# ZechengLi19/CIM

Hardware: AMD Instinct MI355X
Metric: images/sec training step (ResNet-50 VOC, ~1k proposals/img) at 1/2/4/8 GPU (higher is better)
Workload: dtype fp32

## Files before the change

cim_amd/_lib.py:

```python
import ctypes
import os

from ctypes import c_float, c_int, c_longlong, c_void_p

HERE = os.path.dirname(os.path.abspath(__file__))
LIB_PATH = os.environ.get("CIM_HIP_LIB") or os.path.join(HERE, "libcim_hip.so")

_P = c_void_p
SIGNATURES = {
    "cim_roi_align_fwd": [_P, _P, _P] + [c_int] * 6 + [c_float, c_int, c_int, _P],
    "cim_roi_align_fwd_ws": [_P, _P, _P] + [c_int] * 6 + [c_float, c_int, c_int, _P, _P],
    "cim_roi_align_maskcat_fwd_ws": [_P, _P, _P, _P] + [c_int] * 6 + [c_float, c_int, c_int, _P, _P],
    "cim_roi_align_wino7_pair_fwd": [_P, _P, _P, _P, _P] + [c_int] * 7 + [c_float, c_int, c_int, _P, _P],
    "cim_roi_align_bwd_ws": [_P, _P, _P] + [c_int] * 6 + [c_float, c_int, c_int, _P, c_int, _P, _P],
    "cim_roi_align_maskcat_bwd_ws": [_P, _P, _P, _P] + [c_int] * 6 + [c_float, c_int, c_int, _P, c_int, _P, _P],
    "cim_roi_align_bwd_workspace": [c_int, c_int, c_int, c_int],
    "cim_roi_align_bwd_scratch": [c_int, c_int, c_int, c_int, c_int],
    "cim_roi_align_bwd": [_P, _P, _P] + [c_int] * 6 + [c_float, c_int, c_int, _P, _P],
    "cim_roi_align_maskcat_fwd": [_P, _P, _P, _P] + [c_int] * 6 + [c_float, c_int, c_int, _P],
    "cim_roi_align_maskcat_bwd": [_P, _P, _P, _P] + [c_int] * 6 + [c_float, c_int, c_int, _P, _P],
    "cim_roi_align_forms": [c_int] * 9 + [_P] * 3,
    "cim_maxpool2d_out_size": [c_int, c_int, c_int, c_int],
    "cim_maxpool2d_fwd": [_P, _P, _P, c_int, c_int, c_int, c_int, c_int, c_int, _P],
    "cim_maxpool2d_bwd": [_P, _P, _P, c_int, c_int, c_int, c_int, c_int, c_int, _P],
    "cim_upsample_nearest_fwd": [_P, _P, c_int, c_int, c_int, c_int, c_int, _P],
    "cim_upsample_nearest_bwd": [_P, _P, c_int, c_int, c_int, c_int, _P],
    "cim_image_prep": [_P, c_int, c_int, _P, c_int, c_int, c_longlong, c_int, ctypes.c_double, c_int, _P, _P],
    "cim_mask_pack": [_P, _P, c_int, c_int, _P],
    "cim_mask_iou_pair": [_P, c_int, c_int, _P, _P, _P, _P],
    "cim_asy_flag": [_P, c_int, c_float, _P, _P],
    "cim_asy_prep": [_P, c_int, _P, c_int, _P, _P, _P],
    "cim_mining_step": [_P, _P, _P],
    "cim_mining_lds_bytes": [c_int, c_int],
    "cim_mining_sync_bytes": [],
    "cim_gemm_small_splits": [c_int, c_int, c_int],
    "cim_gemm_small_f32": [_P, _P, _P] + [c_int] * 8 + [_P, _P, _P, _P, _P, c_float, _P, c_int, c_int, _P, _P],
    "cim_conv1x1_bwd_workspace": [c_int, c_int, c_int, c_int],
    "cim_conv1x1_bn_act_bwd": [_P] * 8 + [c_float, c_int] + [_P] * 5 + [c_int] * 4 + [_P, _P, _P, _P, _P, c_int] + [c_int, _P, _P, c_float] + [_P] * 4 + [c_int],
    "cim_bn_part_finish": [_P, c_int, _P],
    "cim_conv3x3_nchw_splits": [c_int] * 5,
    "cim_conv3x3_nchw_f32": [_P, _P, _P] + [c_int] * 6 + [_P, _P, _P, _P, _P, c_float, _P, c_int, c_int, _P, _P],
    "cim_conv7x7_nchw_f32": [_P, _P, _P] + [c_int] * 5 + [_P, _P, _P, _P, c_float, c_int, _P],
    "cim_conv3x3_nchw_bwd_workspace": [c_int] * 6,
    "cim_conv3x3_dx_parts": [c_int] * 3,
    "cim_conv3x3_nchw_bn_act_bwd": [_P] * 8 + [c_float, c_int] + [_P] * 5 + [c_int] * 7 + [_P, _P, _P, _P, _P, c_int] + [c_int, _P, _P, c_float] + [_P] * 4,
    "cim_conv3x3_wt_multi": [_P, c_int, _P],
    "cim_bn_act_fwd": [_P, _P, _P, _P, _P, _P, c_float, _P, c_int, c_int, c_int, c_int, _P],
    "cim_bn_act_bwd_chunks": [c_int, c_int, c_int],
    "cim_bn_act_bwd": [_P, _P, _P, _P, _P, _P, c_float, _P, _P, _P, _P, c_int, c_int, c_int, c_int, _P],
    "cim_sgd_multi": [_P, _P, c_int, c_float, c_int, _P],
    "cim_adam_multi": [_P, _P, c_int, ctypes.c_double, ctypes.c_double, ctypes.c_double, c_int, _P],
    "cim_gemm_pair_splits": [c_int, c_int, c_int],
    "cim_gemm_pair": [_P, _P, _P, _P] + [c_int] * 6 + [c_int, c_int, c_int, c_int, _P, _P, _P, _P, c_int, c_int, c_int, _P],
    "cim_gemm_pair_batched": [_P, _P, _P] + [c_int] * 6 + [c_int, c_int, c_int, c_longlong, c_longlong, c_longlong,
                              _P, _P, c_int, c_int, c_int, _P],
    "cim_pair_scales": [_P, c_int, _P, _P, c_int, c_int, _P],
    "cim_pair_split": [_P, _P, c_int, c_int, c_int, c_int, c_int, c_int, c_longlong, c_longlong, _P, _P, _P],
    "cim_pair_amax": [_P, c_longlong, _P, _P],
    "cim_pair_masked_stats": [_P, _P, c_int, c_int, _P, _P, _P],
    "cim_wino7_flatten_bwd_dy_pair": [_P, _P, _P, _P, _P, _P, _P, c_int, c_int, c_int, _P],
    "cim_wino7_pair_scales": [_P, c_int, _P, c_int, _P, _P],
    "cim_wino7_input_pair": [_P, _P, _P, c_int, c_int, c_int, _P],
    "cim_wino7_filter_pair": [_P, _P, _P, c_int, c_int, _P],
    "cim_wino7_dy_pair": [_P, _P, _P, c_int, c_int, c_int, c_int, _P],
    "cim_wino7_output_amax": [_P, _P, _P, c_int, c_int, c_int, _P, _P],
    "cim_flatten_chw_pair": [_P, _P, _P, c_int, c_int, c_int, c_int, _P],
    "cim_flatten_chw_bwd_bias": [_P, _P, _P, _P, c_int, c_int, c_int, _P],
    "cim_wino_dx_adjoint_output": [_P, _P, c_int, c_int, c_int, c_int, _P],
    "cim_wino7_dx_maskfold": [_P, _P, _P, c_int, c_int, _P],
    "cim_wino_wgrad_output": [_P, _P, c_int, c_int, c_int, _P],
    "cim_losses_fwd": [_P, _P],
    "cim_linear_bias_f32": [_P, _P, _P, _P, c_int, c_int, c_int, c_int, _P, _P],
    "cim_loss_finish": [_P, c_int, _P, _P],
    "cim_loss_grad_combine": [_P] * 8 + [c_int, c_int, c_int, _P],
    "cim_head_act_fwd": [_P, _P, _P, c_int, c_int, c_int, _P],
    "cim_head_act_bwd": [_P, _P, _P, _P, c_int, c_int, c_int, _P],
    "cim_detect_ws_bytes": [c_int, c_int],
    "cim_detect_nms_limit": [_P, c_int, _P, c_int, c_int, c_float, c_float, c_int, _P, _P, _P, _P, _P],
    "cim_detect_corloc": [_P, c_int, c_int, c_int, _P, _P],
    "cim_segm_words": [c_int, c_int],
    "cim_segm_pack": [_P, _P, c_longlong, c_int, c_int, c_int, _P, _P],
    "cim_segm_area": [_P, c_int, c_int, _P, _P],
    "cim_segm_rle_count": [_P, c_int, c_int, c_int, _P, _P],
    "cim_segm_rle_write": [_P, c_int, c_int, c_int, _P, _P, _P, _P],
    "cim_segm_rle_decode_ws_bytes": [c_longlong],
    "cim_segm_rle_decode": [_P, _P, _P, c_int, c_int, c_int, _P, _P, _P],
    "cim_segm_image_ws_bytes": [c_int, c_int, c_longlong],
    "cim_segm_record_bytes": [c_int, c_int, c_int, c_int],
    "cim_segm_eval_image": [_P, c_int, _P, c_int, c_int, _P, _P, c_int, c_int, c_int, c_longlong, _P, _P, _P, c_int, _P, c_int,
                            _P, _P, _P],
# ... 77 lines not shown
```

cim_amd/csrc/common.h:

```cpp
#pragma once
#include <hip/hip_runtime.h>
#include <hip/hip_fp16.h>
#include <stdint.h>
#include <stdio.h>

namespace cim {

void set_error(const char* fmt, ...);

static inline hipStream_t as_stream(void* s) { return reinterpret_cast<hipStream_t>(s); }

static inline float round_to_f16(float thr) { return (float)(_Float16)thr; }

#define CIM_CHECK_ARG(cond)                                                     \
    do {                                                                        \
        if (!(cond)) {                                                          \
            cim::set_error("%s: bad argument: %s", __func__, #cond);            \
            return -1;                                                          \
        }                                                                       \
    } while (0)

#define CIM_CHECK_LAUNCH()                                                      \
    do {                                                                        \
        hipError_t e_ = hipGetLastError();                                      \
        if (e_ != hipSuccess) {                                                 \
            cim::set_error("%s: %s", __func__, hipGetErrorString(e_));          \
            return (int)e_;                                                     \
        }                                                                       \
    } while (0)

#define CIM_CHECK_HIP(call)                                                     \
    do {                                                                        \
        hipError_t e_ = (call);                                                 \
        if (e_ != hipSuccess) {                                                 \
            cim::set_error("%s: %s", __func__, hipGetErrorString(e_));          \
            return (int)e_;                                                     \
        }                                                                       \
    } while (0)

typedef _Float16 pair_f16x2 __attribute__((ext_vector_type(2)));
typedef float pair_f32x2 __attribute__((ext_vector_type(2)));
__device__ __forceinline__ void pair_split2(float a, float b, unsigned& h, unsigned& l) {
    const pair_f32x2 v = {a, b};
    const pair_f16x2 hv = __builtin_convertvector(v, pair_f16x2);
    const pair_f32x2 r = {a - (float)hv.x, b - (float)hv.y};
    h = __builtin_bit_cast(unsigned, hv);
    l = __builtin_bit_cast(unsigned, __builtin_convertvector(r, pair_f16x2));
}
__device__ __forceinline__ float pair_scale_of(unsigned amax_bits) {
    const int e = (int)((amax_bits >> 23) & 0xffu);
    int b = 268 - e;
    if (b > 253) b = 253;
    if (e == 0 || e == 255) b = 127;
    return __uint_as_float((unsigned)b << 23);
}

__device__ __forceinline__ void amax_publish(unsigned* word, unsigned wave_max) {
    if (wave_max > __hip_atomic_load(word, __ATOMIC_RELAXED, __HIP_MEMORY_SCOPE_AGENT)) atomicMax(word, wave_max);
}

__device__ __forceinline__ float h2f(uint16_t bits) {
    return __half2float(__ushort_as_half(bits));
}

}
```

cim_amd/csrc/gemm_pair.hip:

```cpp
#include "common.h"
#include <type_traits>
#include "../../include/cim_hip.h"

namespace {

using f32x16 = __attribute__((ext_vector_type(16))) float;
using f16x8 = __attribute__((ext_vector_type(8))) _Float16;
typedef short s16x4 __attribute__((__vector_size__(4 * sizeof(short))));
typedef short s16x8 __attribute__((__vector_size__(8 * sizeof(short))));

#ifndef CIM_PAIR_EXP
#define CIM_PAIR_EXP 0
#endif
static_assert(CIM_PAIR_EXP == 0 || (CIM_PAIR_EXP >= 3 && CIM_PAIR_EXP <= 5), "CIM_PAIR_EXP: 0 (product), 3, 4 or 5");
constexpr bool ABL_NO_LOOP_DMA = CIM_PAIR_EXP == 3 || CIM_PAIR_EXP == 5;
constexpr bool ABL_NO_LOOP_READS = CIM_PAIR_EXP == 4 || CIM_PAIR_EXP == 5;

constexpr int BM = 256, BN = 256, BK = 32;
constexpr int NW = 8, NT = 64 * NW;
constexpr int WNC = 4;
constexpr int WM = 128, WN = BN / WNC, MI = 4, NI = WN / 32;
constexpr int IPW = 32 / NW;
constexpr int OPER = 256 * BK * 4;
constexpr int SLAB = 2 * OPER;
// ... 578 lines not shown
using cim::pair_split2;
using cim::pair_scale_of;

__global__ __launch_bounds__(256) void pair_masked_stats_kernel(const float* __restrict__ dy, const float* __restrict__ y, int rows,
                                                                int cols, float* __restrict__ part, unsigned* __restrict__ amax) {
    __shared__ float4 red[16][16];
    const int cx = threadIdx.x & 15, ry = threadIdx.x >> 4;
    const int col = blockIdx.x * 64 + cx * 4, r0 = blockIdx.y * 64;
    float4 s = make_float4(0.f, 0.f, 0.f, 0.f);
    unsigned m = 0;
    if (col < cols) {
#pragma unroll
        for (int i = 0; i < 4; ++i) {
            const int r = r0 + ry * 4 + i;
            if (r < rows) {
                const float4 g = *reinterpret_cast<const float4*>(dy + (size_t)r * cols + col);
                const float4 v = *reinterpret_cast<const float4*>(y + (size_t)r * cols + col);
                const float4 z = make_float4(v.x > 0.f ? g.x : 0.f, v.y > 0.f ? g.y : 0.f, v.z > 0.f ? g.z : 0.f, v.w > 0.f ? g.w : 0.f);
                s.x += z.x; s.y += z.y; s.z += z.z; s.w += z.w;
                m = max(m, abs_bits_max4(z));
            }
        }
    }
    if (part != nullptr) red[ry][cx] = s;
    block_amax_publish(amax, m);
    if (part == nullptr) return;
    if (ry == 0 && col < cols) {
        float4 t = red[0][cx];
#pragma unroll
        for (int k = 1; k < 16; ++k) { const float4 u = red[k][cx]; t.x += u.x; t.y += u.y; t.z += u.z; t.w += u.w; }
        *reinterpret_cast<float4*>(part + (size_t)blockIdx.y * cols + col) = t;
    }
}
__global__ void pair_scales_kernel(const unsigned* __restrict__ amax, int n_amax, const float* __restrict__ factor,
                                   float* __restrict__ scale, int n, int reduce_all) {
    const int i = blockIdx.x * blockDim.x + threadIdx.x;
    unsigned bits = 0;
    if (reduce_all) {
        for (int t = threadIdx.x & 63; t < n_amax; t += 64) bits = max(bits, amax[t] & 0x7fffffffu);
        bits = wave_max_u32(bits);
    }
    if (i >= n) return;
    float a = __uint_as_float(reduce_all ? bits : amax[min(i, n_amax - 1)]);
    if (factor != nullptr) a *= factor[i];
    scale[i] = pair_scale_of(__float_as_uint(a));
}

__global__ __launch_bounds__(256) void pair_split_kernel(const float* __restrict__ X, char* __restrict__ P, int rows,
                                                         int rows_pad, int cols, int ld, int ldp, long long x_bs,
                                                         long long p_bs, const float* __restrict__ scale,
                                                         const float* __restrict__ relu_y) {
    const int chunks = cols >> 3;
    const long long idx = (long long)blockIdx.x * 256 + threadIdx.x;
    if (idx >= (long long)rows_pad * chunks) return;
    const int r = (int)(idx / chunks), c = (int)(idx % chunks);
    const int z = blockIdx.y;
    uint4 h = make_uint4(0, 0, 0, 0), l = make_uint4(0, 0, 0, 0);
    if (r < rows) {
        const float s = scale[z];
        const float* src = X + (size_t)z * x_bs + (size_t)r * ld + c * 8;
        float4 a = *reinterpret_cast<const float4*>(src), b = *reinterpret_cast<const float4*>(src + 4);
        if (relu_y != nullptr) {
            const float* ys = relu_y + (size_t)z * x_bs + (size_t)r * ld + c * 8;
            const float4 ya = *reinterpret_cast<const float4*>(ys), yb = *reinterpret_cast<const float4*>(ys + 4);
            a = make_float4(ya.x > 0.f ? a.x : 0.f, ya.y > 0.f ? a.y : 0.f, ya.z > 0.f ? a.z : 0.f, ya.w > 0.f ? a.w : 0.f);
            b = make_float4(yb.x > 0.f ? b.x : 0.f, yb.y > 0.f ? b.y : 0.f, yb.z > 0.f ? b.z : 0.f, yb.w > 0.f ? b.w : 0.f);
        }
        pair_split2(a.x * s, a.y * s, h.x, l.x);
        pair_split2(a.z * s, a.w * s, h.y, l.y);
        pair_split2(b.x * s, b.y * s, h.z, l.z);
        pair_split2(b.z * s, b.w * s, h.w, l.w);
    }
    char* dst = P + ((size_t)z * p_bs + (size_t)r * ldp + c * 8) * 4;
    *reinterpret_cast<uint4*>(dst) = h;
    *reinterpret_cast<uint4*>(dst + 16) = l;
}

__global__ __launch_bounds__(256) void pair_amax_kernel(const float* __restrict__ X, long long n4, int tail, unsigned* __restrict__ out) {
    unsigned m = 0;
    if (blockIdx.x == 0 && (int)threadIdx.x < tail) m = abs_bits(X[n4 * 4 + threadIdx.x]);
    for (long long i = (long long)blockIdx.x * 256 + threadIdx.x; i < n4; i += (long long)gridDim.x * 256) {
        const uint4 v = *reinterpret_cast<const uint4*>(X + i * 4);
        m = max(m, abs_bits_max4(v));
    }
    block_amax_publish(out, m);
}

template <int AL, int BL, bool RING>
int launch_pair(PairArgs g, int splits, float* workspace, hipStream_t st, int max_workgroups, int products) {
    static_assert(!RING || (AL == L_MC && BL == L_MC), "the ring kernel is the weight gradients' layout only");
    constexpr int TBM = RING ? RBM : BM, LDSB = RING ? RLDS_BYTES : LDS_BYTES, THREADS = RING ? RNT : NT;
    const int tm = (g.M + TBM - 1) / TBM, tn = (g.N + BN - 1) / BN;
    void (*kern)(const PairArgs);
    if constexpr (RING) kern = products == 1 ? gemm_pair_ring_kernel<true> : gemm_pair_ring_kernel<false>;
    else kern = products == 1 ? gemm_pair_kernel<AL, BL, true> : gemm_pair_kernel<AL, BL, false>;
    hipError_t e = hipFuncSetAttribute(reinterpret_cast<const void*>(kern), hipFuncAttributeMaxDynamicSharedMemorySize, LDSB);
    if (e != hipSuccess) return (int)e;
    const int slabs = g.K / BK;
    if (splits < 1) splits = 1;
    if (splits > slabs) splits = slabs;
    g.k_per_split = ((slabs + splits - 1) / splits) * BK;
    splits = (g.K + g.k_per_split - 1) / g.k_per_split;
    float* out = g.C;
    const float* bias = g.bias;
// ... 101 lines not shown
    if (rc) { cim::set_error("cim_gemm_pair: launch setup failed (%d)", rc); return rc; }
    CIM_CHECK_LAUNCH();
    return 0;
}

extern "C" int cim_gemm_pair_batched(const void* A, const void* B, float* C, int M, int N, int K, int lda, int ldb,
                                     int ldc, int a_mcontig, int b_kcontig, int batch, long long a_bs, long long b_bs,
                                     long long c_bs, const float* a_scale, const float* b_scale, int max_workgroups, int products,
                                     int form, void* stream) {
    CIM_CHECK_ARG(A && B && C && a_scale && b_scale && batch > 0 && batch <= 65535 && max_workgroups >= 0 && (products == 3 || products == 1));
    CIM_CHECK_ARG(form == 0 || (form == 1 && a_mcontig && !b_kcontig));
    CIM_CHECK_ARG(pair_dims_ok(M, N, K, lda, ldb, ldc, a_mcontig, b_kcontig));
    CIM_CHECK_ARG(a_bs % 8 == 0 && b_bs % 8 == 0 && c_bs % 4 == 0);
    PairArgs g = pair_args(A, B, C, M, N, K, lda, ldb, ldc, a_scale, b_scale);
    g.batch = batch;
    g.a_bs = a_bs;
    g.b_bs = b_bs;
    g.c_bs = c_bs;
    int rc = dispatch_pair(g, a_mcontig, b_kcontig, 1, nullptr, cim::as_stream(stream), max_workgroups, products, form);
    if (rc) { cim::set_error("cim_gemm_pair_batched: launch setup failed (%d)", rc); return rc; }
    CIM_CHECK_LAUNCH();
    return 0;
}

extern "C" int cim_pair_scales(const uint32_t* amax, int n_amax, const float* factor, float* scale, int n, int reduce_all, void* stream) {
    CIM_CHECK_ARG(amax && scale && n > 0 && n_amax > 0);
    hipLaunchKernelGGL(pair_scales_kernel, dim3((n + 255) / 256), dim3(256), 0, cim::as_stream(stream), amax, n_amax, factor, scale, n,
                       reduce_all);
    CIM_CHECK_LAUNCH();
    return 0;
}

extern "C" int cim_pair_split(const float* X, void* P, int rows, int rows_pad, int cols, int ld, int ldp, int batch,
                              long long x_bs, long long p_bs, const float* scale, const float* relu_y, void* stream) {
    CIM_CHECK_ARG(X && P && scale && rows > 0 && rows_pad >= rows && cols > 0 && batch > 0 && batch <= 65535);
    CIM_CHECK_ARG(cols % 8 == 0 && ld % 4 == 0 && ld >= cols && ldp % 8 == 0 && ldp >= cols && x_bs % 4 == 0 && p_bs % 8 == 0);
    const long long chunks = (long long)rows_pad * (cols / 8);
    hipLaunchKernelGGL(pair_split_kernel, dim3((unsigned)((chunks + 255) / 256), batch), dim3(256), 0, cim::as_stream(stream), X,
                       (char*)P, rows, rows_pad, cols, ld, ldp, x_bs, p_bs, scale, relu_y);
    CIM_CHECK_LAUNCH();
    return 0;
}

extern "C" int cim_pair_masked_stats(const float* dy, const float* y, int rows, int cols, float* part, uint32_t* amax, void* stream) {
    CIM_CHECK_ARG(dy && y && amax && rows > 0 && cols > 0 && cols % 4 == 0);
    hipLaunchKernelGGL(pair_masked_stats_kernel, dim3((unsigned)((cols + 63) / 64), (unsigned)((rows + 63) / 64)), dim3(256), 0,
                       cim::as_stream(stream), dy, y, rows, cols, part, amax);
    CIM_CHECK_LAUNCH();
    return 0;
}

extern "C" int cim_pair_amax(const float* X, long long n, uint32_t* amax, void* stream) {
    CIM_CHECK_ARG(X && amax && n > 0 && ((size_t)X & 15) == 0);
    const long long n4 = n / 4;
    const unsigned blocks = (unsigned)((n4 + 256 * 8 - 1) / (256 * 8) < 2048 ? (n4 + 256 * 8 - 1) / (256 * 8) : 2048);
    hipLaunchKernelGGL(pair_amax_kernel, dim3(blocks ? blocks : 1), dim3(256), 0, cim::as_stream(stream), X, n4, (int)(n - n4 * 4), amax);
    CIM_CHECK_LAUNCH();
    return 0;
}
```

cim_amd/csrc/sgd.hip:

```cpp
#include "common.h"
#include "../../include/cim_hip.h"
#include "optim_stream.h"

namespace {

__device__ __forceinline__ float4 sgd_update4(float4& pv, const float4& gv, float4& bv, float momentum, float lr, float wd) {
    bv.x = fmaf(momentum, bv.x, fmaf(wd, pv.x, gv.x));
    bv.y = fmaf(momentum, bv.y, fmaf(wd, pv.y, gv.y));
    bv.z = fmaf(momentum, bv.z, fmaf(wd, pv.z, gv.z));
    bv.w = fmaf(momentum, bv.w, fmaf(wd, pv.w, gv.w));
    pv.x = fmaf(-lr, bv.x, pv.x);
    pv.y = fmaf(-lr, bv.y, pv.y);
    pv.z = fmaf(-lr, bv.z, pv.z);
    pv.w = fmaf(-lr, bv.w, pv.w);
    return pv;
}

__global__ __launch_bounds__(256) void sgd_multi_kernel(const cim_sgd_tensor* __restrict__ tensors,
                                                        const cim_sgd_chunk* __restrict__ chunks, int n_chunks, float momentum) {
  for (int ci = blockIdx.x; ci < n_chunks; ci += gridDim.x) {
    const cim_sgd_chunk ch = chunks[ci];
    const cim_sgd_tensor t = tensors[ch.tensor];
    const float lr = t.lr, wd = t.wd;
    if (t.cols > 0) {
        const int r0 = (int)ch.offset, r1 = min((int)t.rows, r0 + 64);
        const int c = ch.n + threadIdx.x * 4;
        const bool cin = c < t.cols;
        const size_t base = (size_t)r0 * t.cols + (cin ? c : 0);
        float* __restrict__ p = reinterpret_cast<float*>(t.p) + base;
        const float* __restrict__ g = reinterpret_cast<const float*>(t.g) + base;
        float* __restrict__ b = reinterpret_cast<float*>(t.buf) + base;
        unsigned* row_amax = reinterpret_cast<unsigned*>(t.row_amax);
        unsigned* col_amax = reinterpret_cast<unsigned*>(t.col_amax);
        const bool lead = (threadIdx.x & 63) == 63;
        uint4 cm = make_uint4(0, 0, 0, 0);
        const size_t ld = (size_t)t.cols;
        int r = r0;
        for (; r + 4 <= r1; r += 4, p += 4 * ld, g += 4 * ld, b += 4 * ld) {
            float4 pv[4], gv[4], bv[4];
            unsigned m[4] = {0, 0, 0, 0};
            if (cin) {
#pragma unroll
                for (int i = 0; i < 4; ++i) {
                    pv[i] = sgd_load(p + i * ld);
                    gv[i] = sgd_load(g + i * ld);
                    bv[i] = sgd_load(b + i * ld);
                }
#pragma unroll
                for (int i = 0; i < 4; ++i) {
                    sgd_update4(pv[i], gv[i], bv[i], momentum, lr, wd);
                    sgd_store(b + i * ld, bv[i]);
                    sgd_store(p + i * ld, pv[i]);
                    const unsigned ax = __float_as_uint(pv[i].x) & 0x7fffffffu, ay = __float_as_uint(pv[i].y) & 0x7fffffffu;
                    const unsigned az = __float_as_uint(pv[i].z) & 0x7fffffffu, aw = __float_as_uint(pv[i].w) & 0x7fffffffu;
                    cm.x = max(cm.x, ax); cm.y = max(cm.y, ay); cm.z = max(cm.z, az); cm.w = max(cm.w, aw);
                    m[i] = max(max(ax, ay), max(az, aw));
                }
            }
#pragma unroll
            for (int i = 0; i < 4; ++i) {
                const unsigned mm = sgd_wave_max(m[i]);
                if (lead) atomicMax(row_amax + r + i, mm);
            }
        }
        for (; r < r1; ++r, p += ld, g += ld, b += ld) {
            unsigned m = 0;
            if (cin) {
                float4 pv = sgd_load(p);
                const float4 gv = sgd_load(g);
                float4 bv = sgd_load(b);
                sgd_update4(pv, gv, bv, momentum, lr, wd);
                sgd_store(b, bv);
                sgd_store(p, pv);
                const unsigned ax = __float_as_uint(pv.x) & 0x7fffffffu, ay = __float_as_uint(pv.y) & 0x7fffffffu;
                const unsigned az = __float_as_uint(pv.z) & 0x7fffffffu, aw = __float_as_uint(pv.w) & 0x7fffffffu;
                cm.x = max(cm.x, ax); cm.y = max(cm.y, ay); cm.z = max(cm.z, az); cm.w = max(cm.w, aw);
                m = max(max(ax, ay), max(az, aw));
            }
            m = sgd_wave_max(m);
            if (lead) atomicMax(row_amax + r, m);
        }
        if (cin) {
            atomicMax(col_amax + c, cm.x); atomicMax(col_amax + c + 1, cm.y);
            atomicMax(col_amax + c + 2, cm.z); atomicMax(col_amax + c + 3, cm.w);
        }
        continue;
    }
    float* __restrict__ p = reinterpret_cast<float*>(t.p) + ch.offset;
    const float* __restrict__ g = reinterpret_cast<const float*>(t.g) + ch.offset;
    float* __restrict__ b = reinterpret_cast<float*>(t.buf) + ch.offset;
    const int n = min(ch.n, (int)(t.n - ch.offset));
    const bool aligned = ((t.p | t.g | t.buf) & 15) == 0;
    const int n4 = aligned ? (n & ~3) : 0;
    for (int i = threadIdx.x * 4; i < n4; i += 256 * 4) {
        float4 pv = *reinterpret_cast<const float4*>(p + i);
        const float4 gv = *reinterpret_cast<const float4*>(g + i);
        float4 bv = *reinterpret_cast<const float4*>(b + i);
        sgd_update4(pv, gv, bv, momentum, lr, wd);
        *reinterpret_cast<float4*>(b + i) = bv;
        *reinterpret_cast<float4*>(p + i) = pv;
    }
    for (int i = n4 + threadIdx.x; i < n; i += 256) {
        const float bv = fmaf(momentum, b[i], fmaf(wd, p[i], g[i]));
        b[i] = bv;
        p[i] = fmaf(-lr, bv, p[i]);
    }
  }
}

}

extern "C" int cim_sgd_multi(const cim_sgd_tensor* tensors, const cim_sgd_chunk* chunks, int n_chunks, float momentum,
                             int max_workgroups, void* stream) {
    CIM_CHECK_ARG((tensors != nullptr && chunks != nullptr) || n_chunks == 0);
    CIM_CHECK_ARG(n_chunks >= 0 && max_workgroups >= 0);
    if (n_chunks == 0) return 0;
    const int grid = max_workgroups > 0 && max_workgroups < n_chunks ? max_workgroups : n_chunks;
// ... 5 lines not shown
```

cim_amd/ops/maskfuse_pair.py:

```python
import torch
from torch.autograd import Function

from .. import _lib
from . import chain
from . import gemm as G
from . import pair

NPOS = 121
DEFER_DW = True
DW_WGS = 256
DW_FORM = 1
DW_FORM1_WGS = 0
import collections as _collections
SCHEDULE = _collections.Counter()


def supported(cat, wc, w1, w2):
    r, cin, p, q = cat.shape
    cout = wc.shape[0]
    return (cat.is_cuda and p == 7 and q == 7 and cin % 32 == 0 and cout % 64 == 0 and wc.shape[1] == cin
            and w1.shape[1] == cout * 49 and w1.shape[0] % 32 == 0 and w2.shape[1] == w1.shape[0] and w2.shape[0] % 32 == 0)


def _weight_amax(w, rows, cols):
# ... 6 lines not shown
_IMAGES = {}
import weakref as _weakref


def _store(w, img, ev):
    key = id(w)
    _IMAGES[key] = (w._version, w.data_ptr(), img, ev, _weakref.ref(w, lambda _r, key=key: _IMAGES.pop(key, None)))


_STALE_FC = False


def _cached(w):
    e = _IMAGES.get(id(w))
    if e is not None and e[4]() is w and ((e[0] == w._version and e[1] == w.data_ptr()) or (_STALE_FC and w.dim() == 2)):
        return e
    return None


def _conv_image(w):
    cout, cin = w.shape[0], w.shape[1]
    sc = torch.empty(NPOS, dtype=torch.float32, device=w.device)
    st = _lib.stream_ptr()
    wa = _weight_amax(w, cout, cin * 9)
    _lib.call("cim_wino7_pair_scales", wa.data_ptr(), wa.numel(), None, 1, sc.data_ptr(), st)
    U = pair.Pair(torch.empty((NPOS, cout, cin), dtype=torch.int32, device=w.device), cout, cin, NPOS, sc)
    _lib.call("cim_wino7_filter_pair", w.data_ptr(), U.buf.data_ptr(), sc.data_ptr(), cout, cin, st)
    return U


def _fc_image(w):
    n, k = w.shape
    return pair.split(w.detach(), n, k, k, scale=pair.scales_from(_weight_amax(w, n, k), 1, reduce_all=True))


def weight_image(w, conv=False):
    e = _cached(w)
    if e is not None:
        if e[3] is not None:
            torch.cuda.current_stream(w.device).wait_event(e[3])
            e[2].record_stream(torch.cuda.current_stream(w.device))
        return e[2]
    G.wait_pending_updates(w.device)
    with torch.no_grad():
        img = _conv_image(w.contiguous()) if conv else _fc_image(w.contiguous())
    _store(w, img, None)
    return img


FUSE_DY = True
PREFETCH = True


def prefetch_weight_images(wc, w1, w2):
    if not (G.OVERLAP and PREFETCH and wc.is_cuda) or torch.cuda.is_current_stream_capturing():
        return
    todo = [(w, c) for w, c in ((wc, True), (w1, False), (w2, False)) if _cached(w) is None and w.is_contiguous()]
    if not todo:
        return
    dev = wc.device
    cur, side = torch.cuda.current_stream(dev), G._side_stream(dev)
    side.wait_stream(cur)
    with torch.cuda.stream(side), torch.no_grad():
        for w, conv in todo:
            img = _conv_image(w) if conv else _fc_image(w)
            ev = torch.cuda.Event()
# ... 317 lines not shown
```

cim_amd/ops/pair.py:

```python
import torch

from .. import _lib


def pad32(n):
    return (n + 31) & ~31


class Pair:
    __slots__ = ("buf", "rows", "cols", "batch", "scale")

    def __init__(self, buf, rows, cols, batch, scale):
        self.buf, self.rows, self.cols, self.batch, self.scale = buf, rows, cols, batch, scale

    @property
    def rows_pad(self):
        return self.buf.shape[-2]

    @property
    def ld(self):
        return self.buf.shape[-1]

    @property
    def bs(self):
# ... 14 lines not shown


def masked_stats(dy, y, amax, want_colsum, reduce=True):
    rows, cols = dy.shape
    part = torch.empty(((rows + 63) // 64, cols), dtype=torch.float32, device=dy.device) if want_colsum else None
    _lib.call("cim_pair_masked_stats", dy.data_ptr(), y.data_ptr(), rows, cols, _lib.ptr(part), amax.data_ptr(), _lib.stream_ptr())
    if not want_colsum:
        return None
    return part.sum(dim=0) if reduce else part


def scales_from(amax, n=1, factor=None, reduce_all=False):
    s = torch.empty(n, dtype=torch.float32, device=amax.device)
    _lib.call("cim_pair_scales", amax.data_ptr(), amax.numel(), _lib.ptr(factor), s.data_ptr(), n, int(reduce_all), _lib.stream_ptr())
    return s


def empty(rows, cols, batch, dev, scale=None, zero_pad=True):
    rp = pad32(rows)
    buf = torch.empty((batch, rp, cols), dtype=torch.int32, device=dev)
    if zero_pad and rp != rows:
        buf[:, rows:, :].zero_()
    return Pair(buf, rows, cols, batch, scale)


def split(x, rows=None, cols=None, ld=None, batch=1, x_bs=0, scale=None, relu_y=None):
    if rows is None:
        rows, cols = x.shape[-2], x.shape[-1]
        ld = cols
    if scale is None:
        scale = scales_from(amax_of(x), batch)
    p = empty(rows, cols, batch, x.device, scale, zero_pad=False)
    _lib.call("cim_pair_split", x.data_ptr(), p.buf.data_ptr(), rows, p.rows_pad, cols, ld, cols, batch, x_bs, p.bs,
              scale.data_ptr(), _lib.ptr(relu_y), _lib.stream_ptr())
    return p


def tail_columns(m, n, k):
    tm, tn = (m + 255) // 256, (n + 255) // 256
    total = tm * tn
    if total <= 256 or total % 256 == 0 or n % 256:
        return None
    main_tn = tn
    while main_tn > 0 and (main_tn * tm) % 256:
        main_tn -= 1
    tail = (tn - main_tn) * tm
    if main_tn == 0 or tail > 64:
        return None
    s = 1
    while s * 2 * tail <= 256 and k // (s * 2 * 32) >= 8 and s < 16:
        s *= 2
    return (main_tn * 256, s) if s > 1 else None


def tail_entries(m, n, k, batch):
    t = ((m + 255) // 256) * ((n + 255) // 256)
    rem = (batch * t) % 256
    if batch * t <= 256 or rem == 0 or rem > 64 or rem % t:
        return None
    s = 1
    while s * 2 * t <= 256 and k // (s * 2 * 32) >= 8 and s < 16:
        s *= 2
    return (rem // t, s) if s > 1 else None


PRODUCTS = 3

# ... 39 lines not shown
```

cim_amd/optim/fused.py:

```python
import numpy as np
import torch

from ..ops.gemm import join_side as _join_side

from .. import _lib

CHUNK = 16384
_CHUNK = np.dtype([("tensor", "<i4"), ("n", "<i4"), ("offset", "<i8")])
MATRIX_MIN = 1 << 20
TRAIL_MIN = 1 << 24
TILE_ROWS, TILE_COLS = 64, 1024


def _matrix_shape(p):
    if p.dim() < 2 or p.numel() < MATRIX_MIN:
        return None
    rows = p.shape[0]
    cols = p.numel() // rows
    return (rows, cols) if cols % 4 == 0 else None


class _Pass:

    def __init__(self):
# ... 114 lines not shown
            stale = stale or self._pointers_moved(c)
            if not stale and self._check_every_step:
                n_sel = sum(1 for g in self.param_groups for p in g["params"] if p.grad is not None and select(p))
                stale = n_sel != len(grads)
            if stale:
                c = None
        if c is None:
            if not self._scan(ps, select):
                return
            c = ps.cache
            grads = [p.grad for p, _, _ in c["recs"]]
        tab, dev = c["tab"], c["dev"]
        keep, gp = [], []
        for g in grads:
            if g.dtype != torch.float32 or not g.is_contiguous():
                if g.dtype != torch.float32 or g.is_sparse:
                    raise NotImplementedError(self._NAME + ": dense fp32 gradients")
                g = g.contiguous()
                keep.append(g)
            gp.append(g.data_ptr())
        tab["g"] = gp
        if any(gp[i] & 15 for i, _, _, _ in c["amax_off"]):
            ps.cache = None
            if not _retry:
                raise _lib.CimHipError(self._NAME + ": inconsistent gradient alignment")
            return self._run(key, select, _retry=False)
        self._fill(tab, c)
        amax_buf = torch.zeros(max(c["n_amax"], 1), dtype=torch.int32, device=dev)
        base = amax_buf.data_ptr()
        slices = []
        for i, off, rows, cols in c["amax_off"]:
            tab["row_amax"][i], tab["col_amax"][i] = base + 4 * off, base + 4 * (off + rows)
            slices.append((c["recs"][i][0], amax_buf[off:off + rows], amax_buf[off + rows:off + rows + cols], rows, cols))
        raw = tab.view(np.uint8).reshape(-1)
        sig = raw.tobytes()
        if sig != c["sig"]:
            if c["copied"] is not None:
                c["copied"].synchronize()
            c["pinned"].numpy()[:] = raw
            c["table"].copy_(c["pinned"], non_blocking=True)
            c["copied"] = torch.cuda.Event()
            c["copied"].record()
            c["sig"] = sig
        self._launch(c, ps, self.trail_workgroups if key == "trail" else 0)
        torch.autograd.graph.increment_version(c["touched"])
        if slices:
            from ..ops import gemm
            for p, ra, ca, rows, cols in slices:
                gemm.register_weight_scales(p, rows, cols, ra, ca)
        return c["ids"]

    def _invalidate(self):
        for ps in self._passes.values():
            ps.cache = None

    def load_state_dict(self, state_dict):
        super().load_state_dict(state_dict)
        self._invalidate()

    def __setstate__(self, state):
        super().__setstate__(state)
        self.__dict__.setdefault("_passes", {})
        self.__dict__.setdefault("_early", None)
        self.__dict__.setdefault("_check_every_step", True)
        self._invalidate()

    def add_param_group(self, param_group):
        super().add_param_group(param_group)
        if hasattr(self, "_passes"):
            self._invalidate()

    def _before_launches(self):
        """Called at the top of step() and step_early(), before anything is enqueued."""

    @torch.no_grad()
    def step_early(self, params, stream):
        self._before_launches()
        ids = frozenset(id(p) for p in params)
        cur = torch.cuda.current_stream()
        stream.wait_stream(cur)
        with torch.cuda.stream(stream):
            done = self._run("early", lambda p: id(p) in ids)
# ... 59 lines not shown
```

cim_amd/optim/sgd.py:

```python
import numpy as np
import torch

from .. import _lib
from .fused import CHUNK, MATRIX_MIN, TILE_COLS, TILE_ROWS, TRAIL_MIN, FusedOptimizer, _matrix_shape, _Pass

_TENSOR = np.dtype([("p", "<u8"), ("g", "<u8"), ("buf", "<u8"), ("n", "<i8"), ("lr", "<f4"), ("wd", "<f4"),
                    ("rows", "<i4"), ("cols", "<i4"), ("row_amax", "<u8"), ("col_amax", "<u8")])


class SGD(FusedOptimizer):
    _NAME = "cim_amd.optim.SGD"
    _RECORD = _TENSOR
    _STATE = (("buf", "momentum_buffer"),)

    def __init__(self, params, lr=1e-3, momentum=0.0, dampening=0.0, weight_decay=0.0, nesterov=False):
        if dampening != 0.0 or nesterov:
            raise NotImplementedError("cim_amd.optim.SGD: dampening / Nesterov are not used by the reference and not provided")
        defaults = dict(lr=lr, momentum=momentum, dampening=dampening, weight_decay=weight_decay, nesterov=nesterov)
        super().__init__(params, defaults)

    def _rule(self):
        momentum = None
        for group in self.param_groups:
            if group.get("dampening", 0.0) != 0.0 or group.get("nesterov", False):
                raise NotImplementedError("cim_amd.optim.SGD: dampening / Nesterov")
            if momentum is None:
                momentum = float(group["momentum"])
            elif float(group["momentum"]) != momentum:
                raise NotImplementedError("cim_amd.optim.SGD: one momentum value for all groups")
        return momentum

    def _new_state(self, p, st):
        if st.get("momentum_buffer") is None:
            st["momentum_buffer"] = torch.zeros_like(p, memory_format=torch.contiguous_format)

    def _fill(self, tab, c):
        lrs = np.array([float(g["lr"]) for g in self.param_groups], dtype=np.float32)
        wds = np.array([float(g["weight_decay"]) for g in self.param_groups], dtype=np.float32)
        tab["lr"], tab["wd"] = lrs[c["group_of"]], wds[c["group_of"]]

# ... 3 lines not shown
```

include/cim_hip.h:

```cpp
#ifndef CIM_HIP_H
#define CIM_HIP_H

#include <stdint.h>

#ifdef __cplusplus
extern "C" {
#endif

const char* cim_last_error(void);
int cim_abi_version(void);

int cim_roi_align_fwd(const float* feat, const float* rois, float* out,
                      int B, int C, int H, int W, int K, int P,
                      float spatial_scale, int sampling_ratio, int aligned, void* stream);

long long cim_roi_align_bwd_workspace(int K, int P, int H, int W);
int cim_roi_align_bwd(const float* grad_out, const float* rois, float* grad_in,
                      int B, int C, int H, int W, int K, int P,
                      float spatial_scale, int sampling_ratio, int aligned, float* workspace, void* stream);

int cim_roi_align_fwd_ws(const float* feat, const float* rois, float* out,
                         int B, int C, int H, int W, int K, int P,
                         float spatial_scale, int sampling_ratio, int aligned, float* workspace, void* stream);
int cim_roi_align_maskcat_fwd_ws(const float* feat, const float* rois, const float* masks, float* cat,
// ... 152 lines not shown
                         const float* residual, int relu, int splits, float* workspace, void* stream);
int cim_conv7x7_nchw_f32(const float* x, const float* w, float* y, int cin, int cout, int H, int W, int stride,
                         const float* gamma, const float* beta, const float* mean, const float* var, float eps, int relu,
                         void* stream);
long long cim_conv3x3_nchw_bwd_workspace(int B, int cin, int cout, int H, int W, int stride);
int cim_conv3x3_dx_parts(int H, int W, int stride);
int cim_conv3x3_nchw_bn_act_bwd(const float* dy, const float* y, const float* x_raw, const float* x, const float* w,
                                const float* gamma, const float* mean, const float* var, float eps, int relu, float* dres,
                                float* dgamma, float* dbeta, float* dx, float* dw, int B, int cin, int cout, int H, int W,
                                int stride, int dilation, float* workspace, void* stream, void* side_stream, void* fork_event,
                                void* join_event, int join, int dy_is_dconv, const float* in_gamma, const float* in_var, float in_eps,
                                const float* in_xr, const float* in_mean, float* in_part, const float* wt_ready);
typedef struct { const float* w; float* wt; int cin; int cout; } cim_wt_desc;
int cim_conv3x3_wt_multi(const cim_wt_desc* descs, int n, void* stream);

int cim_bn_act_fwd(const float* x, const float* res, const float* gamma, const float* beta, const float* mean,
                   const float* var, float eps, float* y, int N, int C, int HW, int relu, void* stream);
int cim_bn_act_bwd_chunks(int N, int C, int HW);
int cim_bn_act_bwd(const float* dy, const float* y, const float* x, const float* gamma, const float* mean,
                   const float* var, float eps, float* dx, float* dres, float* dgamma, float* dbeta,
                   int N, int C, int HW, int relu, void* stream);

int cim_gemm_pair_splits(int M, int N, int K);
int cim_gemm_pair(const void* A, const void* B, float* C, const float* bias, int M, int N, int K,
                  int lda, int ldb, int ldc, int a_mcontig, int b_kcontig, int relu, int splits, float* workspace,
                  const float* a_scale, const float* b_scale, uint32_t* c_amax, int max_workgroups, int products, int form,
                  void* stream);
int cim_gemm_pair_batched(const void* A, const void* B, float* C, int M, int N, int K,
                          int lda, int ldb, int ldc, int a_mcontig, int b_kcontig,
                          int batch, long long a_bs, long long b_bs, long long c_bs,
                          const float* a_scale, const float* b_scale, int max_workgroups, int products, int form, void* stream);
int cim_pair_scales(const uint32_t* amax, int n_amax, const float* factor, float* scale, int n, int reduce_all, void* stream);
int cim_pair_split(const float* X, void* P, int rows, int rows_pad, int cols, int ld, int ldp, int batch,
                   long long x_bs, long long p_bs, const float* scale, const float* relu_y, void* stream);
int cim_pair_amax(const float* X, long long n, uint32_t* amax, void* stream);
int cim_pair_masked_stats(const float* dy, const float* y, int rows, int cols, float* part, uint32_t* amax, void* stream);

int cim_wino7_pair_scales(const uint32_t* amax, int n_amax, const uint32_t* amax_mul, int kind, float* scale, void* stream);
int cim_wino7_input_pair(const float* x, void* V, const float* scale, int R, int Rs, int C, void* stream);
int cim_wino7_filter_pair(const float* W, void* U, const float* scale, int Cout, int Cin, void* stream);
int cim_wino7_dy_pair(const float* dy, void* D, const float* scale, int R, int Rs, int C, int adjoint, void* stream);
int cim_wino7_flatten_bwd_dy_pair(const float* dX, const float* relu_y, void* E, const float* scale_e, void* D, const float* scale_d,
                                  float* bias_partial, int R, int Rs, int C, void* stream);
int cim_wino7_output_amax(const float* M, const float* bias, float* y, int R, int C, int relu, uint32_t* y_amax, void* stream);
int cim_flatten_chw_pair(const float* src, void* dst, const float* scale, int R, int Rs, int PP, int C, void* stream);
int cim_flatten_chw_bwd_bias(const float* src, const float* relu_y, float* dst, float* bias_partial, int R, int PP, int C,
                             void* stream);


int cim_wino_wgrad_output(const float* dU, float* dW, int Cout, int Cin, int tile, void* stream);
int cim_wino_dx_adjoint_output(const float* M, float* dx, int R, int P, int C, int tile, void* stream);
int cim_wino7_dx_maskfold(const float* M, const float* masks, float* dbox, int R, int Cb, void* stream);

#define CIM_PCL_MAX_CLUSTERS 256
typedef struct cim_loss_args {
    const float* pc;
    const float* pd;
    const float* rc[3];
    const float* ri[3];
    const float* pseudo_labels[3];
    const uint16_t* pseudo_iou_f16[3];
    const float* loss_weights[3];
    float weight_scale[3];
    const int32_t* layer_valid;
    const float* labels;
    const float* mat;
    int32_t* status;
    int N, C1, R;
    float* part;
    float* grad;
    int ld;
} cim_loss_args;

int cim_losses_fwd(const cim_loss_args* args, void* stream);

int cim_linear_bias_f32(const float* X, const float* W, const float* bias, float* Y, int M, int N, int K, int splits,
                        float* workspace, void* stream);
int cim_loss_finish(const float* part, int rows, float* out, void* stream);
int cim_loss_grad_combine(const float* G, const float* g_bag, const float* g_pcl, const float* g_cls, const float* g_iou,
                          const float* g_iou3, const float* g_total, float* out, int N, int C1, int R, void* stream);
int cim_head_act_fwd(const float* logits, float* scores, float* colstat, int N, int C1, int R, void* stream);
int cim_head_act_bwd(const float* scores, const float* grad_scores, float* grad_logits, float* coldot,
                     int N, int C1, int R, void* stream);

typedef struct cim_sgd_tensor {
    uint64_t p;
    uint64_t g;
    uint64_t buf;
    int64_t n;
    float lr, wd;
    int32_t rows, cols;
    uint64_t row_amax, col_amax;
} cim_sgd_tensor;
typedef struct cim_sgd_chunk {
    int32_t tensor;
    int32_t n;
    int64_t offset;
} cim_sgd_chunk;
int cim_sgd_multi(const cim_sgd_tensor* tensors, const cim_sgd_chunk* chunks, int n_chunks, float momentum, int max_workgroups,
                  void* stream);

typedef struct cim_adam_tensor {
    uint64_t p;
    uint64_t g;
    uint64_t exp_avg;
    uint64_t exp_avg_sq;
    int64_t n;
    float step_size, bc2_sqrt, wd;
    int32_t rows, cols;
    int32_t reserved;
    uint64_t row_amax, col_amax;
} cim_adam_tensor;
int cim_adam_multi(const cim_adam_tensor* tensors, const cim_sgd_chunk* chunks, int n_chunks, double beta1, double beta2, double eps,
                   int max_workgroups, void* stream);

#ifdef __cplusplus
}
#endif
#endif
```

Before: 76.69.

## Write fp16 pair weight images directly from the fused SGD update

The fused SGD kernel now also writes the split fp16 hi/lo pair image of each updated FC weight, using a scale predicted from the previous step's registered row amax. A small confirm kernel then recomputes the scale from the new amax, and the pair_split kernel re-splits the weight only if the predicted scale was wrong. This removes a separate read-and-split pass over the weights before the next forward. The cost is extra stores in the optimizer, a host-side speculation path, and the complexity of the fallback.

```diff
diff --git a/cim_amd/_lib.py b/cim_amd/_lib.py
--- a/cim_amd/_lib.py
+++ b/cim_amd/_lib.py
@@ -55,7 +55,8 @@
     "cim_gemm_pair_batched": [_P, _P, _P] + [c_int] * 6 + [c_int, c_int, c_int, c_longlong, c_longlong, c_longlong,
                               _P, _P, c_int, c_int, c_int, _P],
     "cim_pair_scales": [_P, c_int, _P, _P, c_int, c_int, _P],
-    "cim_pair_split": [_P, _P, c_int, c_int, c_int, c_int, c_int, c_int, c_longlong, c_longlong, _P, _P, _P],
+    "cim_pair_split": [_P, _P, c_int, c_int, c_int, c_int, c_int, c_int, c_longlong, c_longlong, _P, _P, _P, _P],
+    "cim_pair_scale_confirm": [_P, c_int, _P, _P, _P, _P],
     "cim_pair_amax": [_P, c_longlong, _P, _P],
     "cim_pair_masked_stats": [_P, _P, c_int, c_int, _P, _P, _P],
     "cim_wino7_flatten_bwd_dy_pair": [_P, _P, _P, _P, _P, _P, _P, c_int, c_int, c_int, _P],
diff --git a/cim_amd/csrc/common.h b/cim_amd/csrc/common.h
--- a/cim_amd/csrc/common.h
+++ b/cim_amd/csrc/common.h
@@ -47,6 +47,10 @@
     h = __builtin_bit_cast(unsigned, hv);
     l = __builtin_bit_cast(unsigned, __builtin_convertvector(r, pair_f16x2));
 }
+__device__ __forceinline__ void pair_split4(const float4& v, float s, unsigned& h0, unsigned& h1, unsigned& l0, unsigned& l1) {
+    pair_split2(v.x * s, v.y * s, h0, l0);
+    pair_split2(v.z * s, v.w * s, h1, l1);
+}
 __device__ __forceinline__ float pair_scale_of(unsigned amax_bits) {
     const int e = (int)((amax_bits >> 23) & 0xffu);
     int b = 268 - e;
diff --git a/cim_amd/csrc/gemm_pair.hip b/cim_amd/csrc/gemm_pair.hip
--- a/cim_amd/csrc/gemm_pair.hip
+++ b/cim_amd/csrc/gemm_pair.hip
@@ -634,24 +634,35 @@
         *reinterpret_cast<float4*>(part + (size_t)blockIdx.y * cols + col) = t;
     }
 }
+__device__ __forceinline__ unsigned pair_amax_of_all(const unsigned* __restrict__ amax, int n_amax) {
+    unsigned bits = 0;
+    for (int t = threadIdx.x & 63; t < n_amax; t += 64) bits = max(bits, amax[t] & 0x7fffffffu);
+    return wave_max_u32(bits);
+}
 __global__ void pair_scales_kernel(const unsigned* __restrict__ amax, int n_amax, const float* __restrict__ factor,
                                    float* __restrict__ scale, int n, int reduce_all) {
     const int i = blockIdx.x * blockDim.x + threadIdx.x;
     unsigned bits = 0;
-    if (reduce_all) {
-        for (int t = threadIdx.x & 63; t < n_amax; t += 64) bits = max(bits, amax[t] & 0x7fffffffu);
-        bits = wave_max_u32(bits);
-    }
+    if (reduce_all) bits = pair_amax_of_all(amax, n_amax);
     if (i >= n) return;
     float a = __uint_as_float(reduce_all ? bits : amax[min(i, n_amax - 1)]);
     if (factor != nullptr) a *= factor[i];
     scale[i] = pair_scale_of(__float_as_uint(a));
 }
+__global__ void pair_scale_confirm_kernel(const unsigned* __restrict__ amax, int n_amax, const float* __restrict__ spec,
+                                          float* __restrict__ scale, unsigned* __restrict__ ok) {
+    const float s = pair_scale_of(pair_amax_of_all(amax, n_amax));
+    if (threadIdx.x != 0) return;
+    *scale = s;
+    *ok = __float_as_uint(s) == __float_as_uint(*spec) ? 1u : 0u;
+}
 
 __global__ __launch_bounds__(256) void pair_split_kernel(const float* __restrict__ X, char* __restrict__ P, int rows,
                                                          int rows_pad, int cols, int ld, int ldp, long long x_bs,
                                                          long long p_bs, const float* __restrict__ scale,
-                                                         const float* __restrict__ relu_y) {
+                                                         const float* __restrict__ relu_y,
+                                                         const unsigned* __restrict__ skip_if) {
+    if (skip_if != nullptr && *skip_if != 0) return;
     const int chunks = cols >> 3;
     const long long idx = (long long)blockIdx.x * 256 + threadIdx.x;
     if (idx >= (long long)rows_pad * chunks) return;
@@ -668,10 +679,8 @@
             a = make_float4(ya.x > 0.f ? a.x : 0.f, ya.y > 0.f ? a.y : 0.f, ya.z > 0.f ? a.z : 0.f, ya.w > 0.f ? a.w : 0.f);
             b = make_float4(yb.x > 0.f ? b.x : 0.f, yb.y > 0.f ? b.y : 0.f, yb.z > 0.f ? b.z : 0.f, yb.w > 0.f ? b.w : 0.f);
         }
-        pair_split2(a.x * s, a.y * s, h.x, l.x);
-        pair_split2(a.z * s, a.w * s, h.y, l.y);
-        pair_split2(b.x * s, b.y * s, h.z, l.z);
-        pair_split2(b.z * s, b.w * s, h.w, l.w);
+        cim::pair_split4(a, s, h.x, h.y, l.x, l.y);
+        cim::pair_split4(b, s, h.z, h.w, l.z, l.w);
     }
     char* dst = P + ((size_t)z * p_bs + (size_t)r * ldp + c * 8) * 4;
     *reinterpret_cast<uint4*>(dst) = h;
@@ -839,12 +848,20 @@
 }
 
 extern "C" int cim_pair_split(const float* X, void* P, int rows, int rows_pad, int cols, int ld, int ldp, int batch,
-                              long long x_bs, long long p_bs, const float* scale, const float* relu_y, void* stream) {
+                              long long x_bs, long long p_bs, const float* scale, const float* relu_y, const uint32_t* skip_if,
+                              void* stream) {
     CIM_CHECK_ARG(X && P && scale && rows > 0 && rows_pad >= rows && cols > 0 && batch > 0 && batch <= 65535);
     CIM_CHECK_ARG(cols % 8 == 0 && ld % 4 == 0 && ld >= cols && ldp % 8 == 0 && ldp >= cols && x_bs % 4 == 0 && p_bs % 8 == 0);
     const long long chunks = (long long)rows_pad * (cols / 8);
     hipLaunchKernelGGL(pair_split_kernel, dim3((unsigned)((chunks + 255) / 256), batch), dim3(256), 0, cim::as_stream(stream), X,
-                       (char*)P, rows, rows_pad, cols, ld, ldp, x_bs, p_bs, scale, relu_y);
+                       (char*)P, rows, rows_pad, cols, ld, ldp, x_bs, p_bs, scale, relu_y, skip_if);
+    CIM_CHECK_LAUNCH();
+    return 0;
+}
+
+extern "C" int cim_pair_scale_confirm(const uint32_t* amax, int n_amax, const float* spec, float* scale, uint32_t* ok, void* stream) {
+    CIM_CHECK_ARG(amax && spec && scale && ok && n_amax > 0);
+    hipLaunchKernelGGL(pair_scale_confirm_kernel, dim3(1), dim3(64), 0, cim::as_stream(stream), amax, n_amax, spec, scale, ok);
     CIM_CHECK_LAUNCH();
     return 0;
 }
diff --git a/cim_amd/csrc/sgd.hip b/cim_amd/csrc/sgd.hip
--- a/cim_amd/csrc/sgd.hip
+++ b/cim_amd/csrc/sgd.hip
@@ -16,6 +16,19 @@
     return pv;
 }
 
+typedef unsigned sgd_u4 __attribute__((ext_vector_type(4)));
+__device__ __forceinline__ unsigned sgd_swap1(unsigned v) {
+    return (unsigned)__builtin_amdgcn_update_dpp(0, (int)v, 0xB1, 0xf, 0xf, false);
+}
+__device__ __forceinline__ void sgd_store_image(float* q, const float4& v, float s) {
+    unsigned h0, h1, l0, l1;
+    cim::pair_split4(v, s, h0, h1, l0, l1);
+    const bool odd = (threadIdx.x & 1) != 0;
+    const unsigned x0 = sgd_swap1(odd ? h0 : l0), x1 = sgd_swap1(odd ? h1 : l1);
+    const sgd_u4 o = odd ? sgd_u4{x0, x1, l0, l1} : sgd_u4{h0, h1, x0, x1};
+    __builtin_nontemporal_store(o, reinterpret_cast<sgd_u4*>(q));
+}
+
 __global__ __launch_bounds__(256) void sgd_multi_kernel(const cim_sgd_tensor* __restrict__ tensors,
                                                         const cim_sgd_chunk* __restrict__ chunks, int n_chunks, float momentum) {
   for (int ci = blockIdx.x; ci < n_chunks; ci += gridDim.x) {
@@ -32,11 +45,13 @@
         float* __restrict__ b = reinterpret_cast<float*>(t.buf) + base;
         unsigned* row_amax = reinterpret_cast<unsigned*>(t.row_amax);
         unsigned* col_amax = reinterpret_cast<unsigned*>(t.col_amax);
+        float* __restrict__ q = t.img != 0 ? reinterpret_cast<float*>(t.img) + base : nullptr;
+        const float qs = q != nullptr ? *reinterpret_cast<const float*>(t.img_scale) : 0.f;
         const bool lead = (threadIdx.x & 63) == 63;
         uint4 cm = make_uint4(0, 0, 0, 0);
         const size_t ld = (size_t)t.cols;
         int r = r0;
-        for (; r + 4 <= r1; r += 4, p += 4 * ld, g += 4 * ld, b += 4 * ld) {
+        for (; r + 4 <= r1; r += 4, p += 4 * ld, g += 4 * ld, b += 4 * ld, q += q != nullptr ? 4 * ld : 0) {
             float4 pv[4], gv[4], bv[4];
             unsigned m[4] = {0, 0, 0, 0};
             if (cin) {
@@ -51,6 +66,7 @@
                     sgd_update4(pv[i], gv[i], bv[i], momentum, lr, wd);
                     sgd_store(b + i * ld, bv[i]);
                     sgd_store(p + i * ld, pv[i]);
+                    if (q != nullptr) sgd_store_image(q + i * ld, pv[i], qs);
                     const unsigned ax = __float_as_uint(pv[i].x) & 0x7fffffffu, ay = __float_as_uint(pv[i].y) & 0x7fffffffu;
                     const unsigned az = __float_as_uint(pv[i].z) & 0x7fffffffu, aw = __float_as_uint(pv[i].w) & 0x7fffffffu;
                     cm.x = max(cm.x, ax); cm.y = max(cm.y, ay); cm.z = max(cm.z, az); cm.w = max(cm.w, aw);
@@ -63,7 +79,7 @@
                 if (lead) atomicMax(row_amax + r + i, mm);
             }
         }
-        for (; r < r1; ++r, p += ld, g += ld, b += ld) {
+        for (; r < r1; ++r, p += ld, g += ld, b += ld, q += q != nullptr ? ld : 0) {
             unsigned m = 0;
             if (cin) {
                 float4 pv = sgd_load(p);
@@ -72,6 +88,7 @@
                 sgd_update4(pv, gv, bv, momentum, lr, wd);
                 sgd_store(b, bv);
                 sgd_store(p, pv);
+                if (q != nullptr) sgd_store_image(q, pv, qs);
                 const unsigned ax = __float_as_uint(pv.x) & 0x7fffffffu, ay = __float_as_uint(pv.y) & 0x7fffffffu;
                 const unsigned az = __float_as_uint(pv.z) & 0x7fffffffu, aw = __float_as_uint(pv.w) & 0x7fffffffu;
                 cm.x = max(cm.x, ax); cm.y = max(cm.y, ay); cm.z = max(cm.z, az); cm.w = max(cm.w, aw);
@@ -83,6 +100,10 @@
         if (cin) {
             atomicMax(col_amax + c, cm.x); atomicMax(col_amax + c + 1, cm.y);
             atomicMax(col_amax + c + 2, cm.z); atomicMax(col_amax + c + 3, cm.w);
+            if (q != nullptr && r1 == (int)t.rows) {
+                for (int rp = ((int)t.rows + 31) & ~31; r < rp; ++r, q += ld)
+                    __builtin_nontemporal_store(sgd_u4{0, 0, 0, 0}, reinterpret_cast<sgd_u4*>(q));
+            }
         }
         continue;
     }
diff --git a/cim_amd/ops/maskfuse_pair.py b/cim_amd/ops/maskfuse_pair.py
--- a/cim_amd/ops/maskfuse_pair.py
+++ b/cim_amd/ops/maskfuse_pair.py
@@ -62,6 +62,37 @@
 def _fc_image(w):
     n, k = w.shape
     return pair.split(w.detach(), n, k, k, scale=pair.scales_from(_weight_amax(w, n, k), 1, reduce_all=True))
+
+
+UPDATE_IMAGES = True
+
+
+def image_for_update(w, rows, cols):
+    e = _IMAGES.get(id(w))
+    if not UPDATE_IMAGES or e is None or e[4]() is not w or w.dim() != 2 or tuple(w.shape) != (rows, cols) or cols % 8:
+        return None
+    if not w.is_contiguous() or torch.cuda.is_current_stream_capturing():
+        return None
+    reg = G._registered_scales(w, rows, cols)
+    if reg is None or reg[0] is None or not reg[0].is_contiguous() or reg[0].numel() > 65536:
+        return None
+    spec = pair.scales_from(reg[0].reshape(-1), 1, reduce_all=True)
+    img = pair.empty(rows, cols, 1, w.device, torch.empty(1, dtype=torch.float32, device=w.device), zero_pad=False)
+    return img, spec
+
+
+def confirm_update_image(w, img, spec, row_amax):
+    rows, cols = w.shape
+    ok = torch.empty(1, dtype=torch.int32, device=w.device)
+    st = _lib.stream_ptr()
+    _lib.call("cim_pair_scale_confirm", row_amax.data_ptr(), row_amax.numel(), spec.data_ptr(), img.scale.data_ptr(), ok.data_ptr(), st)
+    _lib.call("cim_pair_split", w.data_ptr(), img.buf.data_ptr(), rows, img.rows_pad, cols, cols, cols, 1, 0, img.bs,
+              img.scale.data_ptr(), None, ok.data_ptr(), st)
+    ev = torch.cuda.Event()
+    ev.record(torch.cuda.current_stream(w.device))
+    _store(w, img, ev)
+    SCHEDULE["weight_images_written_by_update"] += 1
+    return ok
 
 
 def weight_image(w, conv=False):
diff --git a/cim_amd/ops/pair.py b/cim_amd/ops/pair.py
--- a/cim_amd/ops/pair.py
+++ b/cim_amd/ops/pair.py
@@ -70,7 +70,7 @@
         scale = scales_from(amax_of(x), batch)
     p = empty(rows, cols, batch, x.device, scale, zero_pad=False)
     _lib.call("cim_pair_split", x.data_ptr(), p.buf.data_ptr(), rows, p.rows_pad, cols, ld, cols, batch, x_bs, p.bs,
-              scale.data_ptr(), _lib.ptr(relu_y), _lib.stream_ptr())
+              scale.data_ptr(), _lib.ptr(relu_y), None, _lib.stream_ptr())
     return p
 
 
diff --git a/cim_amd/optim/fused.py b/cim_amd/optim/fused.py
--- a/cim_amd/optim/fused.py
+++ b/cim_amd/optim/fused.py
@@ -170,6 +170,15 @@
         for i, off, rows, cols in c["amax_off"]:
             tab["row_amax"][i], tab["col_amax"][i] = base + 4 * off, base + 4 * (off + rows)
             slices.append((c["recs"][i][0], amax_buf[off:off + rows], amax_buf[off + rows:off + rows + cols], rows, cols))
+        images = []
+        if "img" in tab.dtype.names:
+            from ..ops import maskfuse_pair
+            tab["img"], tab["img_scale"] = 0, 0
+            for (i, _, rows, cols), (p, ra, _, _, _) in zip(c["amax_off"], slices):
+                got = maskfuse_pair.image_for_update(p, rows, cols)
+                if got is not None:
+                    tab["img"][i], tab["img_scale"][i] = got[0].buf.data_ptr(), got[1].data_ptr()
+                    images.append((p, ra) + got)
         raw = tab.view(np.uint8).reshape(-1)
         sig = raw.tobytes()
         if sig != c["sig"]:
@@ -186,6 +195,8 @@
             from ..ops import gemm
             for p, ra, ca, rows, cols in slices:
                 gemm.register_weight_scales(p, rows, cols, ra, ca)
+        for p, ra, img, spec in images:
+            maskfuse_pair.confirm_update_image(p, img, spec, ra)
         return c["ids"]
 
     def _invalidate(self):
diff --git a/cim_amd/optim/sgd.py b/cim_amd/optim/sgd.py
--- a/cim_amd/optim/sgd.py
+++ b/cim_amd/optim/sgd.py
@@ -5,7 +5,7 @@
 from .fused import CHUNK, MATRIX_MIN, TILE_COLS, TILE_ROWS, TRAIL_MIN, FusedOptimizer, _matrix_shape, _Pass
 
 _TENSOR = np.dtype([("p", "<u8"), ("g", "<u8"), ("buf", "<u8"), ("n", "<i8"), ("lr", "<f4"), ("wd", "<f4"),
-                    ("rows", "<i4"), ("cols", "<i4"), ("row_amax", "<u8"), ("col_amax", "<u8")])
+                    ("rows", "<i4"), ("cols", "<i4"), ("row_amax", "<u8"), ("col_amax", "<u8"), ("img", "<u8"), ("img_scale", "<u8")])
 
 
 class SGD(FusedOptimizer):
diff --git a/include/cim_hip.h b/include/cim_hip.h
--- a/include/cim_hip.h
+++ b/include/cim_hip.h
@@ -208,7 +208,8 @@
                           const float* a_scale, const float* b_scale, int max_workgroups, int products, int form, void* stream);
 int cim_pair_scales(const uint32_t* amax, int n_amax, const float* factor, float* scale, int n, int reduce_all, void* stream);
 int cim_pair_split(const float* X, void* P, int rows, int rows_pad, int cols, int ld, int ldp, int batch,
-                   long long x_bs, long long p_bs, const float* scale, const float* relu_y, void* stream);
+                   long long x_bs, long long p_bs, const float* scale, const float* relu_y, const uint32_t* skip_if, void* stream);
+int cim_pair_scale_confirm(const uint32_t* amax, int n_amax, const float* spec, float* scale, uint32_t* ok, void* stream);
 int cim_pair_amax(const float* X, long long n, uint32_t* amax, void* stream);
 int cim_pair_masked_stats(const float* dy, const float* y, int rows, int cols, float* part, uint32_t* amax, void* stream);
 
@@ -267,6 +268,7 @@
     float lr, wd;
     int32_t rows, cols;
     uint64_t row_amax, col_amax;
+    uint64_t img, img_scale;
 } cim_sgd_tensor;
 typedef struct cim_sgd_chunk {
     int32_t tensor;
```

Result: no change. 76.92, median of 2 (+0.3%).
